# Openflight-sim/OPEN_Ludwig

Measured on AMD Instinct MI355X. Metric: MLUPS (million lattice updates/s) at 256^3 D3Q27; % of HBM roofline, higher is better.
Workload: dtype f32

## Files before the change

open_ludwig_amd/build.py:

```python
from __future__ import annotations

import os
import shutil
import subprocess

_HERE = os.path.dirname(os.path.abspath(__file__))
CSRC = os.path.join(_HERE, "csrc")
SOURCES = ["ludwig_hip.hip"]
DEPENDS = ["ludwig_hip.hip", "kernels.hpp", "all_or_nothing.hpp", "lattice.hpp", "jl_math.h", os.path.join("..", "..", "include", "ludwig_hip.h")]
OUT = os.path.join(CSRC, "libludwig_hip.so")

HIPCC_FLAGS = ["--offload-arch=gfx950", "-O3", "-std=c++17", "-fPIC", "-shared", "-ffp-contract=off",
               "-fno-fast-math", "-Wall", "-Wno-unused-function", "-DLW_NT_STORES"]


def source_digest() -> str:
    import hashlib
    h = hashlib.sha1(" ".join(HIPCC_FLAGS).encode())
    for d in sorted(DEPENDS):
        with open(os.path.join(CSRC, d), "rb") as fh:
            h.update(fh.read())
    return h.hexdigest()[:16]


def hipcc_path() -> str:
    for cand in (shutil.which("hipcc"), "/opt/rocm/bin/hipcc"):
        if cand and os.path.exists(cand):
            return cand
    raise FileNotFoundError("hipcc not found")


def needs_build() -> bool:
    if not os.path.exists(OUT):
        return True
    t = os.path.getmtime(OUT)
    return any(os.path.getmtime(os.path.join(CSRC, d)) > t for d in DEPENDS)


def build_library(force: bool = False, verbose: bool = False, extra_flags=()) -> str:
    if not force and not needs_build():
        return OUT
    cmd = [hipcc_path(), *HIPCC_FLAGS, *extra_flags, *SOURCES, "-o", OUT]
    res = subprocess.run(cmd, cwd=CSRC, capture_output=True, text=True)
    if verbose or res.returncode != 0:
        print(" ".join(cmd))
        print(res.stdout)
        print(res.stderr)
    if res.returncode != 0:
        raise RuntimeError("hipcc failed building libludwig_hip.so")
    return OUT
```

open_ludwig_amd/csrc/kernels.hpp:

```cpp
#pragma once

#include <hip/hip_runtime.h>
#include <stdint.h>
#include <type_traits>

#include "lattice.hpp"
#include "jl_math.h"

namespace lw {

struct SCParams {
    const float *f_in;
    float *f_out;
    float *f_post;
    const uint32_t *post_rows;
    const float *vel_in;
    float *vel_out;
    float *rho;
    const uint8_t *obstacle;
    const float *sponge;
    const float *wall_dist;
    const int32_t *meta;
    const int32_t *items;
    const float *pf_new, *pf_old, *prho_new, *prho_old, *pvel_new, *pvel_old;
// ... 142 lines not shown
    int zs[3];
};

__device__ __forceinline__ NeighbourIds load_neighbour_ids(const int32_t *__restrict__ meta, int z)
{
    int nb[27];
#pragma unroll
    for (int d = 0; d < 27; ++d) nb[d] = meta[d];
    NeighbourIds n;
    const bool z_lo = z == 0, z_hi = z == 7;
#pragma unroll
    for (int j = 0; j < 9; ++j) {
        const int lo = nb[j], mid = nb[9 + j], hi = nb[18 + j];
        n.id[0][j] = z_lo ? lo : mid;
        n.id[1][j] = mid;
        n.id[2][j] = z_hi ? hi : mid;
    }
    n.zs[0] = (z - 1) & 7; n.zs[1] = z; n.zs[2] = (z + 1) & 7;
    return n;
}

struct LanePos {
    int x, y;
    bool x0, x7, y0, y7;
};

template <int K>
__device__ __forceinline__ int source_block(const NeighbourIds &n, const LanePos &l)
{
    constexpr int cx = CX(K), cy = CY(K), g = 1 - CZ(K);
    const bool xo = cx == 1 ? l.x0 : (cx == -1 ? l.x7 : false);
    const bool yo = cy == 1 ? l.y0 : (cy == -1 ? l.y7 : false);
    const int c00 = n.id[g][4], cX = n.id[g][4 - cx], cY = n.id[g][4 - 3 * cy], cXY = n.id[g][4 - cx - 3 * cy];
    int sel = c00;
    if constexpr (cx != 0 && cy != 0) sel = xo ? (yo ? cXY : cX) : (yo ? cY : c00);
    else if constexpr (cx != 0) sel = xo ? cX : c00;
    else if constexpr (cy != 0) sel = yo ? cY : c00;
    return sel;
}
constexpr int SUBGRID_NO_OP1 = 0, SUBGRID_NO_DENOM = 1, SUBGRID_FLOOR = 2, SUBGRID_MODEL = 3;
struct WaleState {
    float nu_eddy, s2;
    int code;
};
__device__ __forceinline__ WaleState wale_state(float g11, float g12, float g13, float g21, float g22, float g23, float g31, float g32,
                                                float g33, float c_wale, float nu_bg)
{
    const float gsq11 = g11 * g11 + g12 * g21 + g13 * g31;
    const float gsq12 = g11 * g12 + g12 * g22 + g13 * g32;
    const float gsq13 = g11 * g13 + g12 * g23 + g13 * g33;
    const float gsq21 = g21 * g11 + g22 * g21 + g23 * g31;
    const float gsq22 = g21 * g12 + g22 * g22 + g23 * g32;
    const float gsq23 = g21 * g13 + g22 * g23 + g23 * g33;
    const float gsq31 = g31 * g11 + g32 * g21 + g33 * g31;
    const float gsq32 = g31 * g12 + g32 * g22 + g33 * g32;
    const float gsq33 = g31 * g13 + g32 * g23 + g33 * g33;

    const float tr_gsq = gsq11 + gsq22 + gsq33;
    const float tr_term = tr_gsq / 3.0f;
    const float Sd11 = gsq11 - tr_term, Sd22 = gsq22 - tr_term, Sd33 = gsq33 - tr_term;
    const float Sd12 = 0.5f * (gsq12 + gsq21), Sd13 = 0.5f * (gsq13 + gsq31), Sd23 = 0.5f * (gsq23 + gsq32);
    const float S12 = 0.5f * (g12 + g21), S13 = 0.5f * (g13 + g31), S23 = 0.5f * (g23 + g32);
    const float OP1 = Sd11 * Sd11 + Sd22 * Sd22 + Sd33 * Sd33 + 2.0f * (Sd12 * Sd12 + Sd13 * Sd13 + Sd23 * Sd23);
    const float OP2 = g11 * g11 + g22 * g22 + g33 * g33 + 2.0f * (S12 * S12 + S13 * S13 + S23 * S23);

    WaleState w;
    w.code = SUBGRID_NO_OP1;
    float nu_eddy = 0.0f;
    if (OP1 > 1.0e-12f) {
        const float OP1_32 = OP1 * sqrtf(OP1);
        const float OP2_52 = OP2 * OP2 * sqrtf(jl_max(OP2, 1.0e-12f));
        const float denom = OP2_52 + OP1 * sqrtf(sqrtf(jl_max(OP1, 1.0e-12f)));
        w.code = SUBGRID_NO_DENOM;
        if (denom > 1.0e-12f) {
            nu_eddy = (c_wale * c_wale) * OP1_32 / denom;
            w.code = nu_eddy > nu_bg ? SUBGRID_MODEL : SUBGRID_FLOOR;
        }
    }
    w.nu_eddy = jl_max(nu_eddy, nu_bg);
    w.s2 = 2.0f * OP2;
    return w;
}

template <int K>
__device__ __forceinline__ float collide_value(float rho, float ux_eq, float uy_eq, float uz_eq, float Pi_xx, float Pi_yy, float Pi_zz,
                                               float Pi_xy, float Pi_yz, float Pi_zx, float one_m_omega)
{
    constexpr int cx = CX(K), cy = CY(K), cz = CZ(K);
    constexpr float w_k = WEIGHT(K);
    constexpr float cx_f = (float)cx, cy_f = (float)cy, cz_f = (float)cz;
    const float usq_eq = ux_eq * ux_eq + uy_eq * uy_eq + uz_eq * uz_eq;
    const float cu = cdot<K>(ux_eq, uy_eq, uz_eq);
    const float feq = rho * w_k * (1.0f + 3.0f * cu + 4.5f * cu * cu - 1.5f * usq_eq);
    constexpr float Q_xx = cx_f * cx_f - CS2_PHYSICS, Q_yy = cy_f * cy_f - CS2_PHYSICS, Q_zz = cz_f * cz_f - CS2_PHYSICS;
    float od = 0.0f;
    bool od_empty = true;
    acc_signed<cx * cy>(od, od_empty, Pi_xy);
    acc_signed<cy * cz>(od, od_empty, Pi_yz);
    acc_signed<cz * cx>(od, od_empty, Pi_zx);
    float inner = Pi_xx * Q_xx + Pi_yy * Q_yy + Pi_zz * Q_zz;
    if constexpr (cx * cy != 0 || cy * cz != 0 || cz * cx != 0) inner = inner + 2.0f * od;
    const float f_neq_reg = (w_k * 4.5f) * inner;
    return feq + one_m_omega * f_neq_reg;
}

constexpr int R_COMP = 11;
constexpr uint32_t R_PLANE_BYTES = R_COMP * 64 * 4, R_BLOCK_BYTES = 8 * R_PLANE_BYTES;
enum { R_RHO, R_UX, R_UY, R_UZ, R_PXX, R_PYY, R_PZZ, R_PXY, R_PYZ, R_PZX, R_OMO };

__device__ __forceinline__ const char *record_plane(const float *base, int blk, int z)
{
    return reinterpret_cast<const char *>(base) + (uint64_t)(uint32_t)blk * R_BLOCK_BYTES + (uint32_t)z * R_PLANE_BYTES;
}
__device__ __forceinline__ void load_record(float (&r)[R_COMP], const char *plane, uint32_t lane4)
{
    const float *q = reinterpret_cast<const float *>(plane + lane4);
#pragma unroll
    for (int c = 0; c < R_COMP; ++c) r[c] = q[c * 64];
}
template <bool WIDE>
using record_off_t = std::conditional_t<WIDE, uint64_t, uint32_t>;
template <bool WIDE>
__device__ __forceinline__ record_off_t<WIDE> record_offset(int blk, int z)
{
    return (record_off_t<WIDE>)(uint32_t)blk * R_BLOCK_BYTES + (uint32_t)z * R_PLANE_BYTES;
}
template <class OFF>
__device__ __forceinline__ void load_record_at(float (&r)[R_COMP], const float *base, OFF off)
{
    const float *q = reinterpret_cast<const float *>(reinterpret_cast<const char *>(base) + off);
#pragma unroll
    for (int c = 0; c < R_COMP; ++c) r[c] = q[c * 64];
}
__device__ __forceinline__ void store_record(float *base, const Own own, float rho, float ux, float uy, float uz, float Pi_xx, float Pi_yy,
                                             float Pi_zz, float Pi_xy, float Pi_yz, float Pi_zx, float one_m_omega)
{
    char *plane = const_cast<char *>(record_plane(base, own.b, __builtin_amdgcn_readfirstlane((int)(own.cell4 >> 8))));
    float *q = reinterpret_cast<float *>(plane + (own.cell4 & 255u));
    const float v[R_COMP] = {rho, ux, uy, uz, Pi_xx, Pi_yy, Pi_zz, Pi_xy, Pi_yz, Pi_zx, one_m_omega};
#pragma unroll
    for (int c = 0; c < R_COMP; ++c) {
#ifdef LW_NT_STORES
        __builtin_nontemporal_store(v[c], q + c * 64);
#else
        q[c * 64] = v[c];
#endif
    }
}
template <int CY_, int CZ_>
__device__ __forceinline__ void record_row(float (&fs)[Q], const float (&r)[R_COMP])
{
    static_for<0, 3>([&](auto ic) {
        constexpr int k = decltype(ic)::value + 3 * (CY_ + 1) + 9 * (CZ_ + 1);
        fs[k] = collide_value<k>(r[R_RHO], r[R_UX], r[R_UY], r[R_UZ], r[R_PXX], r[R_PYY], r[R_PZZ], r[R_PXY], r[R_PYZ], r[R_PZX], r[R_OMO]);
    });
}
template <int CY_, int CZ_>
__device__ __forceinline__ float record_face(const float (&r)[R_COMP], bool plus)
{
    constexpr int k = 2 + 3 * (CY_ + 1) + 9 * (CZ_ + 1);
    return collide_value<k>(r[R_RHO], plus ? r[R_UX] : -r[R_UX], r[R_UY], r[R_UZ], r[R_PXX], r[R_PYY], r[R_PZZ],
                            plus ? r[R_PXY] : -r[R_PXY], r[R_PYZ], plus ? r[R_PZX] : -r[R_PZX], r[R_OMO]);
}

template <bool POST, bool WALL, bool REC_OUT = false>
__device__ __forceinline__ void finish_cell(const SCParams &p, const int flags, const Own own, float (&fs)[Q],
                                            const float ux_E, const float uy_E, const float uz_E, const float ux_W, const float uy_W, const float uz_W,
                                            const float ux_N, const float uy_N, const float uz_N, const float ux_S, const float uy_S, const float uz_S,
                                            const float ux_T, const float uy_T, const float uz_T, const float ux_B, const float uy_B, const float uz_B)
{
    float rho = 0.0f, jx = 0.0f, jy = 0.0f, jz = 0.0f;
    static_for<0, Q>([&](auto kc) {
        constexpr int k = decltype(kc)::value;
        constexpr int cx = CX(k), cy = CY(k), cz = CZ(k);
        const float val = fs[k];
        rho += val;
        if constexpr (cx == 1) jx += val; else if constexpr (cx == -1) jx -= val;
        if constexpr (cy == 1) jy += val; else if constexpr (cy == -1) jy -= val;
        if constexpr (cz == 1) jz += val; else if constexpr (cz == -1) jz -= val;
    });

    bool store_post = false;
    if constexpr (POST) {
        if (flags & FLAG_STORE_POST) {
            store_post = true;
            if (p.post_rows) {
                const int zu = __builtin_amdgcn_readfirstlane((int)(own.cell4 >> 8));
                const uint32_t w = p.post_rows[(size_t)own.b * 2 + (zu >> 2)];
                store_post = ((w >> ((zu & 3) * 8 + ((own.cell4 >> 5) & 7))) & 1u) != 0;
            }
        }
    }
    bool is_obs = false;
    if (flags & FLAG_HAS_OBSTACLE) is_obs = p.obstacle[(size_t)own.b * CELLS + (own.cell4 >> 2)] != 0;
    if (is_obs) {
        st_f32(p.vel_out, own.b, V_BLOCK_BYTES, own.cell4, 0.0f);
        st_f32(p.vel_out, own.b, V_BLOCK_BYTES, COMP_BYTES + own.cell4, 0.0f);
        st_f32(p.vel_out, own.b, V_BLOCK_BYTES, 2 * COMP_BYTES + own.cell4, 0.0f);
        if (p.rho_old_save) st_f32(p.rho_old_save, own.b, S_BLOCK_BYTES, own.cell4, ld_own(p.rho, own.b, S_BLOCK_BYTES, own.cell4));
        if (p.store_rho) st_f32(p.rho, own.b, S_BLOCK_BYTES, own.cell4, 1.0f);
        static_for<0, Q>([&](auto kc) {
            constexpr int k = decltype(kc)::value;
            const float f_coll = fs[OPP(k)];
            st_f32(p.f_out, own.b, F_BLOCK_BYTES, k * COMP_BYTES + own.cell4, f_coll);
            if constexpr (POST) { if (store_post) st_f32(p.f_post, own.b, F_BLOCK_BYTES, k * COMP_BYTES + own.cell4, f_coll); }
        });
        return;
    }

    rho = jl_max(rho, 0.01f);
    const float inv_rho = 1.0f / rho;
    float ux = jx * inv_rho, uy = jy * inv_rho, uz = jz * inv_rho;

    if (flags & FLAG_HAS_SPONGE) {
        const float sp = ld_own(p.sponge, own.b, S_BLOCK_BYTES, own.cell4);
        if (sp > 0.0f) {
            const float rho_target = 1.0f, ux_target = p.u_inlet;
            rho = rho * (1.0f - sp) + rho_target * sp;
            ux = ux * (1.0f - sp) + ux_target * sp;
            uy = uy * (1.0f - sp);
            uz = uz * (1.0f - sp);
            if (p.sponge_blend == 1) {
                static_for<0, Q>([&](auto kc) {
                    constexpr int k = decltype(kc)::value;
                    const float feq_target = calculate_equilibrium(rho_target, ux_target, 0.0f, 0.0f, WEIGHT(k),
                                                                   (float)CX(k), (float)CY(k), (float)CZ(k));
                    fs[k] = fs[k] * (1.0f - sp) + feq_target * sp;
                });
            }
        }
    }

    float Fx = 0.0f, Fy = 0.0f, Fz = 0.0f;
    float ux_eq = ux, uy_eq = uy, uz_eq = uz;
    if constexpr (WALL) {
        if (flags & FLAG_HAS_NEAR_WALL) {
            const float u_mag = sqrtf(ux * ux + uy * uy + uz * uz);
            const float force_mag = wall_model_force_mag(ld_own(p.wall_dist, own.b, S_BLOCK_BYTES, own.cell4), p.tau, rho, u_mag);
            if (force_mag >= 0.0f) {
                Fx = -force_mag * ux / u_mag;
                Fy = -force_mag * uy / u_mag;
                Fz = -force_mag * uz / u_mag;
            }
        }
        ux_eq = ux + 0.5f * Fx * inv_rho;
        uy_eq = uy + 0.5f * Fy * inv_rho;
        uz_eq = uz + 0.5f * Fz * inv_rho;
    }
    const float usq_eq = ux_eq * ux_eq + uy_eq * uy_eq + uz_eq * uz_eq;

    if constexpr (!REC_OUT) {
        st_f32(p.vel_out, own.b, V_BLOCK_BYTES, own.cell4, ux);
        st_f32(p.vel_out, own.b, V_BLOCK_BYTES, COMP_BYTES + own.cell4, uy);
        st_f32(p.vel_out, own.b, V_BLOCK_BYTES, 2 * COMP_BYTES + own.cell4, uz);
        if (p.rho_old_save) st_f32(p.rho_old_save, own.b, S_BLOCK_BYTES, own.cell4, ld_own(p.rho, own.b, S_BLOCK_BYTES, own.cell4));
        if (p.store_rho) st_f32(p.rho, own.b, S_BLOCK_BYTES, own.cell4, rho);
    }

    const float g11 = 0.5f * (ux_E - ux_W), g12 = 0.5f * (ux_N - ux_S), g13 = 0.5f * (ux_T - ux_B);
    const float g21 = 0.5f * (uy_E - uy_W), g22 = 0.5f * (uy_N - uy_S), g23 = 0.5f * (uy_T - uy_B);
    const float g31 = 0.5f * (uz_E - uz_W), g32 = 0.5f * (uz_N - uz_S), g33 = 0.5f * (uz_T - uz_B);

    const float gsq11 = g11 * g11 + g12 * g21 + g13 * g31;
    const float gsq12 = g11 * g12 + g12 * g22 + g13 * g32;
    const float gsq13 = g11 * g13 + g12 * g23 + g13 * g33;
    const float gsq21 = g21 * g11 + g22 * g21 + g23 * g31;
    const float gsq22 = g21 * g12 + g22 * g22 + g23 * g32;
    const float gsq23 = g21 * g13 + g22 * g23 + g23 * g33;
    const float gsq31 = g31 * g11 + g32 * g21 + g33 * g31;
    const float gsq32 = g31 * g12 + g32 * g22 + g33 * g32;
    const float gsq33 = g31 * g13 + g32 * g23 + g33 * g33;

    const float tr_gsq = gsq11 + gsq22 + gsq33;
    const float tr_term = tr_gsq / 3.0f;
    const float Sd11 = gsq11 - tr_term, Sd22 = gsq22 - tr_term, Sd33 = gsq33 - tr_term;
    const float Sd12 = 0.5f * (gsq12 + gsq21), Sd13 = 0.5f * (gsq13 + gsq31), Sd23 = 0.5f * (gsq23 + gsq32);
    const float S12 = 0.5f * (g12 + g21), S13 = 0.5f * (g13 + g31), S23 = 0.5f * (g23 + g32);
    const float OP1 = Sd11 * Sd11 + Sd22 * Sd22 + Sd33 * Sd33 + 2.0f * (Sd12 * Sd12 + Sd13 * Sd13 + Sd23 * Sd23);
    const float OP2 = g11 * g11 + g22 * g22 + g33 * g33 + 2.0f * (S12 * S12 + S13 * S13 + S23 * S23);

    float nu_eddy = 0.0f;
    if (OP1 > 1.0e-12f) {
        const float OP1_32 = OP1 * sqrtf(OP1);
        const float OP2_52 = OP2 * OP2 * sqrtf(jl_max(OP2, 1.0e-12f));
        const float denom = OP2_52 + OP1 * sqrtf(sqrtf(jl_max(OP1, 1.0e-12f)));
        if (denom > 1.0e-12f) nu_eddy = (p.c_wale * p.c_wale) * OP1_32 / denom;
    }
    nu_eddy = jl_max(nu_eddy, p.nu_bg);
    const float tau_turb = p.tau + nu_eddy * 3.0f;
    const float omega = 1.0f / jl_max(tau_turb, 0.500001f);

    float Pi_xx = 0.0f, Pi_yy = 0.0f, Pi_zz = 0.0f, Pi_xy = 0.0f, Pi_yz = 0.0f, Pi_zx = 0.0f;
    static_for<0, Q>([&](auto kc) {
        constexpr int k = decltype(kc)::value;
        constexpr int cx = CX(k), cy = CY(k), cz = CZ(k);
        const float cu = cdot<k>(ux_eq, uy_eq, uz_eq);
        const float feq = rho * WEIGHT(k) * (1.0f + 3.0f * cu + 4.5f * cu * cu - 1.5f * usq_eq);
        const float f_neq = fs[k] - feq;
        if constexpr (cx != 0) Pi_xx += f_neq;
        if constexpr (cy != 0) Pi_yy += f_neq;
        if constexpr (cz != 0) Pi_zz += f_neq;
        if constexpr (cx * cy == 1) Pi_xy += f_neq; else if constexpr (cx * cy == -1) Pi_xy -= f_neq;
        if constexpr (cy * cz == 1) Pi_yz += f_neq; else if constexpr (cy * cz == -1) Pi_yz -= f_neq;
        if constexpr (cz * cx == 1) Pi_zx += f_neq; else if constexpr (cz * cx == -1) Pi_zx -= f_neq;
    });

    const float one_m_omega = 1.0f - omega;
    const float one_m_half_omega = 1.0f - 0.5f * omega;
    if constexpr (REC_OUT) {
        store_record(p.rec_out, own, rho, ux_eq, uy_eq, uz_eq, Pi_xx, Pi_yy, Pi_zz, Pi_xy, Pi_yz, Pi_zx, one_m_omega);
        return;
    }
    static_for<0, Q>([&](auto kc) {
        constexpr int k = decltype(kc)::value;
        float f_coll = collide_value<k>(rho, ux_eq, uy_eq, uz_eq, Pi_xx, Pi_yy, Pi_zz, Pi_xy, Pi_yz, Pi_zx, one_m_omega);
        if constexpr (WALL) {
            constexpr float w_k = WEIGHT(k);
            constexpr float cx_f = (float)CX(k), cy_f = (float)CY(k), cz_f = (float)CZ(k);
            const float cu = cdot<k>(ux_eq, uy_eq, uz_eq);
            const float force_term = (w_k * 3.0f) * ((cx_f - ux + 3.0f * cu * cx_f) * Fx + (cy_f - uy + 3.0f * cu * cy_f) * Fy +
                                                     (cz_f - uz + 3.0f * cu * cz_f) * Fz);
            f_coll = f_coll + one_m_half_omega * force_term;
        }
        if constexpr (POST) { if (store_post) st_f32(p.f_post, own.b, F_BLOCK_BYTES, k * COMP_BYTES + own.cell4, f_coll); }
        st_f32(p.f_out, own.b, F_BLOCK_BYTES, k * COMP_BYTES + own.cell4, f_coll);
    });
}

__device__ __forceinline__ void finish_rho_only(const SCParams &p, const int flags, const Own own, const float (&fs)[Q])
{
    float rho = 0.0f;
    static_for<0, Q>([&](auto kc) { rho += fs[decltype(kc)::value]; });
    bool is_obs = false;
    if (flags & FLAG_HAS_OBSTACLE) is_obs = p.obstacle[(size_t)own.b * CELLS + (own.cell4 >> 2)] != 0;
    if (is_obs) { st_f32(p.rho, own.b, S_BLOCK_BYTES, own.cell4, 1.0f); return; }
    rho = jl_max(rho, 0.01f);
    if (flags & FLAG_HAS_SPONGE) {
        const float sp = ld_own(p.sponge, own.b, S_BLOCK_BYTES, own.cell4);
        if (sp > 0.0f) rho = rho * (1.0f - sp) + 1.0f * sp;
    }
    st_f32(p.rho, own.b, S_BLOCK_BYTES, own.cell4, rho);
}

__device__ __forceinline__ void patch_missing_sources(const SCParams &p, const int32_t *__restrict__ meta, const NeighbourIds &nbr,
                                                      const LanePos &l, const int z, const Own own, float (&fs)[Q])
{
    const int gx = (meta[NBR_BX] - 1) * BS + l.x + 1, gy = (meta[NBR_BY] - 1) * BS + l.y + 1, gz = (meta[NBR_BZ] - 1) * BS + z + 1;
    const float *iface_own = p.is_level_1 == 0 ? p.f_iface + (size_t)meta[NBR_GBI] * CELLS + (own.cell4 >> 2) : nullptr;
    static_for<0, Q>([&](auto kc) {
        constexpr int k = decltype(kc)::value;
        constexpr int cx = CX(k), cy = CY(k), cz = CZ(k);
        if constexpr (k != 13) {
            if (source_block<k>(nbr, l) < 0) {
                const int src_gx = gx - cx, src_gy = gy - cy, src_gz = gz - cz;
                const bool is_inlet = src_gx < 1, is_outlet = src_gx > p.nx_g;
                const bool is_y_min = src_gy < 1, is_y_max = src_gy > p.ny_g;
                const bool is_z_min = src_gz < 1, is_z_max = src_gz > p.nz_g;
                float val;
                if (is_inlet) {
                    const float noise = p.inlet_turbulence > 0.0f
                                            ? gradient_noise(gy, gz, p.seed, 1234) * p.inlet_turbulence * p.u_inlet
                                            : 0.0f;
                    const float u_inst = p.u_inlet + noise;
                    const float cu_in = (float)cx * u_inst;
                    val = WEIGHT(k) * (1.0f + 3.0f * cu_in + 4.5f * cu_in * cu_in - 1.5f * u_inst * u_inst);
                } else if (is_outlet) {
                    const float cu_out = (float)cx * p.u_inlet;
                    val = WEIGHT(k) * (1.0f + 3.0f * cu_out + 4.5f * cu_out * cu_out - 1.5f * p.u_inlet * p.u_inlet);
                } else if (is_y_min && p.is_symmetric == 1) {
                    val = ld_own(p.f_in, own.b, F_BLOCK_BYTES, MIRROR_Y(k) * COMP_BYTES + own.cell4);
                } else if (is_y_min || is_y_max) {
                    val = ld_own(p.f_in, own.b, F_BLOCK_BYTES, MIRROR_Y(k) * COMP_BYTES + own.cell4);
                } else if (is_z_min || is_z_max) {
                    val = ld_own(p.f_in, own.b, F_BLOCK_BYTES, MIRROR_Z(k) * COMP_BYTES + own.cell4);
                } else if (p.is_level_1 == 0) {
                    val = iface_own[(size_t)k * p.n_iface_blocks * CELLS];
                } else {
                    val = WEIGHT(k);
                }
                fs[k] = val;
            }
        }
    });
}

__device__ __forceinline__ float dpp_from_lower_lane(float v)
{
    return __int_as_float(__builtin_amdgcn_update_dpp(__float_as_int(v), __float_as_int(v), 0x111, 0xF, 0xF, false));
// ... 95 lines not shown
            if (l.x7) xch[wave][18 + c][l.y] = uc[c];
            if (l.x0) xch[wave][21 + c][l.y] = uc[c];
        }
    }
    }
    __syncthreads();
    if (!active) return;
    const int wlo = first ? 0 : wave - 1, whi = last ? NW - 1 : wave + 1;
    static_for<0, Q>([&](auto kc) {
        constexpr int k = decltype(kc)::value;
        constexpr int cx = CX(k);
        if constexpr (cx == 1) {
            const float inner = dpp_from_lower_lane(fs[k]);
            const float edge = first ? halo[k] : xch[wlo][XSLOT(k)][l.y];
            fs[k] = l.x0 ? edge : inner;
        }
        if constexpr (cx == -1) {
            const float inner = dpp_from_upper_lane(fs[k]);
            const float edge = last ? halo[k] : xch[whi][XSLOT(k)][l.y];
            fs[k] = l.x7 ? edge : inner;
        }
    });
    const bool needs_patch = GENERAL && (flags & FLAG_ALL_NEIGHBOURS) == 0;
    if constexpr (RHO_ONLY) {
        if constexpr (GENERAL) { if (needs_patch) patch_missing_sources(p, meta, nbr, l, z, own, fs); }
        finish_rho_only(p, flags, own, fs);
        return;
    }
    float uE[3], uW[3], uN[3], uS[3];
#pragma unroll
    for (int c = 0; c < 3; ++c) {
        const float e_edge = last ? ux_edge_hi[c] : xch[whi][21 + c][l.y];
        const float w_edge = first ? ux_edge_lo[c] : xch[wlo][18 + c][l.y];
        const float e_in = dpp_from_upper_lane(uc[c]), w_in = dpp_from_lower_lane(uc[c]);
        uE[c] = l.x7 ? e_edge : e_in;
        uW[c] = l.x0 ? w_edge : w_in;
        const float n_in = __shfl_down(uc[c], 8, 64), s_in = __shfl_up(uc[c], 8, 64);
        uN[c] = l.y7 ? uy_edge[c] : n_in;
        uS[c] = l.y0 ? uy_edge[c] : s_in;
    }
    if constexpr (GENERAL) { if (needs_patch) patch_missing_sources(p, meta, nbr, l, z, own, fs); }
    finish_cell<POST, WALL, REC_OUT>(p, flags, own, fs, uE[0], uE[1], uE[2], uW[0], uW[1], uW[2], uN[0], uN[1], uN[2], uS[0], uS[1], uS[2],
                                     uT[0], uT[1], uT[2], uB[0], uB[1], uB[2]);
}
template <int NW, bool GENERAL, bool POST, bool WALL, bool RHO_ONLY = false, bool WIDE = false>
__global__ __launch_bounds__(64 * NW) __attribute__((amdgpu_waves_per_eu((WIDE && GENERAL) ? LW_MIN_WAVES - 1 : LW_MIN_WAVES))) void k_stream_collide_xrun(const SCParams p)
{
    stream_collide_xrun<NW, GENERAL, POST, WALL, RHO_ONLY, WIDE, false>(p);
}
template <int NW, bool WIDE>
__global__ __launch_bounds__(64 * NW) __attribute__((amdgpu_waves_per_eu(LW_MIN_WAVES))) void k_records_from_populations(const SCParams p)
{
    stream_collide_xrun<NW, false, false, false, false, WIDE, true>(p);
}

#ifndef LW_REC_WAVES
#define LW_REC_WAVES 4
#endif
#ifndef LW_REC_AHEAD
#define LW_REC_AHEAD 3
#endif
template <int NW, bool WIDE>
__global__ __launch_bounds__(64 * NW) __attribute__((amdgpu_waves_per_eu(LW_REC_WAVES))) void k_step_records(const SCParams p)
{
    __shared__ float xch[NW][24][8];
    const int wave = __builtin_amdgcn_readfirstlane(threadIdx.x >> 6);
    const int raw = p.items[blockIdx.x * NW + wave];
    const bool active = raw >= 0;
    const int item = active ? (raw & ITEM_ID_MASK) : 0;
    const int b = item >> 3;
    const int z = item & 7;
    const int lane = threadIdx.x & 63;
    LanePos l;
    l.x = lane & 7; l.y = lane >> 3;
    l.x0 = l.x == 0; l.x7 = l.x == 7; l.y0 = l.y == 0; l.y7 = l.y == 7;
    const int32_t *__restrict__ meta = p.meta + (size_t)b * NBR_STRIDE;
    const NeighbourIds nbr = load_neighbour_ids(meta, z);
    const Own own{b, (uint32_t)((l.x + 8 * l.y + 64 * z) * 4)};
    const bool first = !active || (raw & ITEM_LINK_W) == 0, last = !active || (raw & ITEM_LINK_E) == 0;
    __shared__ float xedge[NW][2][12][8];
    float fs[Q];
    float uc[3], uT[3], uB[3], uN[3], uS[3];
    if (active) {
    if ((first && l.x0) || (last && l.x7)) {
        float r[9][R_COMP];
        auto load_face = [&](auto jc) {
            constexpr int j = decltype(jc)::value;
            constexpr int cy = j % 3 - 1, g = 1 - (j / 3 - 1);
            const bool yo = cy == 1 ? l.y0 : (cy == -1 ? l.y7 : false);
            const int wX = nbr.id[g][4 - 1], wXY = nbr.id[g][4 - 1 - 3 * cy], eX = nbr.id[g][4 + 1], eXY = nbr.id[g][4 + 1 - 3 * cy];
            const auto oW = record_offset<WIDE>(wX, nbr.zs[g]), oWY = record_offset<WIDE>(wXY, nbr.zs[g]);
            const auto oE = record_offset<WIDE>(eX, nbr.zs[g]), oEY = record_offset<WIDE>(eXY, nbr.zs[g]);
            const auto off = l.x0 ? (yo ? oWY : oW) : (yo ? oEY : oE);
            load_record_at(r[j], p.rec_in, off + (uint32_t)(((l.x0 ? 7 : 0) + 8 * ((l.y - cy) & 7)) * 4));
        };
        static_for<0, LW_REC_AHEAD>(load_face);
        static_for<0, 9>([&](auto jc) {
            constexpr int j = decltype(jc)::value;
            constexpr int cy = j % 3 - 1, cz = j / 3 - 1;
            if constexpr (j + LW_REC_AHEAD < 9) load_face(std::integral_constant<int, j + LW_REC_AHEAD>{});
            __builtin_amdgcn_sched_barrier(0);
            float(&mine)[12][8] = xedge[wave][l.x0 ? 0 : 1];
            mine[j][l.y] = record_face<cy, cz>(r[j], l.x0);
            if constexpr (cy == 0 && cz == 0) { mine[9][l.y] = r[j][R_UX]; mine[10][l.y] = r[j][R_UY]; mine[11][l.y] = r[j][R_UZ]; }
            __builtin_amdgcn_sched_barrier(0);
        });
    }
    {
        float r[9][R_COMP];
        auto load_pulled = [&](auto jc) {
            constexpr int j = decltype(jc)::value;
            constexpr int cy = j % 3 - 1, g = 1 - (j / 3 - 1);
            const uint32_t lane4 = (uint32_t)((l.x + 8 * ((l.y - cy) & 7)) * 4);
            if constexpr (cy == 0) {
                load_record(r[j], record_plane(p.rec_in, nbr.id[g][4], nbr.zs[g]), lane4);
            } else {
                const bool yo = cy == 1 ? l.y0 : l.y7;
                const auto o0 = record_offset<WIDE>(nbr.id[g][4], nbr.zs[g]), oY = record_offset<WIDE>(nbr.id[g][4 - 3 * cy], nbr.zs[g]);
                load_record_at(r[j], p.rec_in, (yo ? oY : o0) + lane4);
            }
        };
        static_for<0, LW_REC_AHEAD>(load_pulled);
        static_for<0, 9>([&](auto jc) {
            constexpr int j = decltype(jc)::value;
            constexpr int cy = j % 3 - 1, cz = j / 3 - 1;
            if constexpr (j + LW_REC_AHEAD < 9) load_pulled(std::integral_constant<int, j + LW_REC_AHEAD>{});
            __builtin_amdgcn_sched_barrier(0);
            const float(&q)[R_COMP] = r[j];
            record_row<cy, cz>(fs, q);
            if constexpr (cy == 0 && cz == 0) { uc[0] = q[R_UX]; uc[1] = q[R_UY]; uc[2] = q[R_UZ]; }
            if constexpr (cy == 0 && cz == 1) { uB[0] = q[R_UX]; uB[1] = q[R_UY]; uB[2] = q[R_UZ]; }
            if constexpr (cy == 0 && cz == -1) { uT[0] = q[R_UX]; uT[1] = q[R_UY]; uT[2] = q[R_UZ]; }
            if constexpr (cy == 1 && cz == 0) { uS[0] = q[R_UX]; uS[1] = q[R_UY]; uS[2] = q[R_UZ]; }
            if constexpr (cy == -1 && cz == 0) { uN[0] = q[R_UX]; uN[1] = q[R_UY]; uN[2] = q[R_UZ]; }
            __builtin_amdgcn_sched_barrier(0);
        });
    }
    static_for<0, Q>([&](auto kc) {
        constexpr int k = decltype(kc)::value;
        constexpr int cx = CX(k);
        if constexpr (cx == 1) { if (l.x7) xch[wave][XSLOT(k)][l.y] = fs[k]; }
        if constexpr (cx == -1) { if (l.x0) xch[wave][XSLOT(k)][l.y] = fs[k]; }
    });
#pragma unroll
    for (int c = 0; c < 3; ++c) {
        if (l.x7) xch[wave][18 + c][l.y] = uc[c];
        if (l.x0) xch[wave][21 + c][l.y] = uc[c];
    }
    }
    __syncthreads();
    if (!active) return;
    const int wlo = first ? 0 : wave - 1, whi = last ? NW - 1 : wave + 1;
    static_for<0, Q>([&](auto kc) {
        constexpr int k = decltype(kc)::value;
        constexpr int cx = CX(k);
        if constexpr (cx == 1) {
            const float inner = dpp_from_lower_lane(fs[k]);
            const float edge = first ? xedge[wave][0][k / 3][l.y] : xch[wlo][XSLOT(k)][l.y];
            fs[k] = l.x0 ? edge : inner;
        }
        if constexpr (cx == -1) {
            const float inner = dpp_from_upper_lane(fs[k]);
            const float edge = last ? xedge[wave][1][k / 3][l.y] : xch[whi][XSLOT(k)][l.y];
            fs[k] = l.x7 ? edge : inner;
        }
    });
    float uE[3], uW[3];
#pragma unroll
    for (int c = 0; c < 3; ++c) {
        const float e_edge = last ? xedge[wave][1][9 + c][l.y] : xch[whi][21 + c][l.y];
        const float w_edge = first ? xedge[wave][0][9 + c][l.y] : xch[wlo][18 + c][l.y];
        const float e_in = dpp_from_upper_lane(uc[c]), w_in = dpp_from_lower_lane(uc[c]);
        uE[c] = l.x7 ? e_edge : e_in;
        uW[c] = l.x0 ? w_edge : w_in;
    }
    finish_cell<false, false, true>(p, 0, own, fs, uE[0], uE[1], uE[2], uW[0], uW[1], uW[2], uN[0], uN[1], uN[2], uS[0], uS[1], uS[2],
                                    uT[0], uT[1], uT[2], uB[0], uB[1], uB[2]);
}

__global__ __launch_bounds__(256) void k_materialise(const SCParams p, int64_t n_cells)
{
    const int64_t i = (int64_t)blockIdx.x * 256 + threadIdx.x;
    if (i >= n_cells) return;
    const int b = (int)(i >> 9);
    const uint32_t cell = (uint32_t)(i & 511);
    float r[R_COMP];
    load_record(r, record_plane(p.rec_in, b, (int)(cell >> 6)), (cell & 63u) * 4);
    const Own own{b, cell * 4};
    st_f32(p.vel_out, b, V_BLOCK_BYTES, own.cell4, r[R_UX]);
    st_f32(p.vel_out, b, V_BLOCK_BYTES, COMP_BYTES + own.cell4, r[R_UY]);
    st_f32(p.vel_out, b, V_BLOCK_BYTES, 2 * COMP_BYTES + own.cell4, r[R_UZ]);
    if (p.rho) st_f32(p.rho, b, S_BLOCK_BYTES, own.cell4, r[R_RHO]);
    static_for<0, Q>([&](auto kc) {
        constexpr int k = decltype(kc)::value;
        st_f32(p.f_out, b, F_BLOCK_BYTES, k * COMP_BYTES + own.cell4,
               collide_value<k>(r[R_RHO], r[R_UX], r[R_UY], r[R_UZ], r[R_PXX], r[R_PYY], r[R_PZZ], r[R_PXY], r[R_PYZ], r[R_PZX], r[R_OMO]));
    });
}

__device__ __forceinline__ float weight_rt(int k)
{
    const int cx = k % 3 - 1, cy = (k / 3) % 3 - 1, cz = k / 9 - 1;
    const int d2 = cx * cx + cy * cy + cz * cz;
    return d2 == 0 ? WEIGHT(13) : d2 == 1 ? WEIGHT(12) : d2 == 2 ? WEIGHT(9) : WEIGHT(0);
}

struct InterfaceArgs {
    const int4 *corners;
    const float4 *weights;
    float4 *mac, *mac2;
    const int4 *links;
    float *f_iface2;
    float tw2;
    int n_sources, n_links;
};

__device__ __forceinline__ float blend_in_time(bool blend, float v_old, float v_new, float tw)
{
    return blend ? v_old * (1.0f - tw) + v_new * tw : v_new;
}

template <bool TWO>
__global__ __launch_bounds__(256) void k_interface_sources(const SCParams p, const InterfaceArgs a)
{
    const int i = blockIdx.x * 256 + threadIdx.x;
    if (i >= a.n_sources) return;
    const int4 c0 = a.corners[2 * i], c1 = a.corners[2 * i + 1];
    const int cc[8] = {c0.x, c0.y, c0.z, c0.w, c1.x, c1.y, c1.z, c1.w};
    const float4 w = a.weights[i];
    const float tw = p.temporal_weight, tw2 = a.tw2;
    const bool blend = p.use_temporal == 1 && tw < 0.99f, blend2 = TWO && p.use_temporal == 1 && tw2 < 0.99f;
    float v1[4][8], v2[4][8];
#pragma unroll
    for (int n = 0; n < 8; ++n) {
        v1[0][n] = 1.0f; v1[1][n] = 0.0f; v1[2][n] = 0.0f; v1[3][n] = 0.0f;
        v2[0][n] = 1.0f; v2[1][n] = 0.0f; v2[2][n] = 0.0f; v2[3][n] = 0.0f;
        if (cc[n] >= 0) {
            const int c = cc[n];
            const size_t cv = (size_t)(c >> 9) * (3 * CELLS) + (c & 511);
            const float vn[4] = {p.prho_new[c], p.pvel_new[cv], p.pvel_new[cv + CELLS], p.pvel_new[cv + 2 * CELLS]};
            float vo[4] = {0.0f, 0.0f, 0.0f, 0.0f};
            if (blend || blend2) { vo[0] = p.prho_old[c]; vo[1] = p.pvel_old[cv]; vo[2] = p.pvel_old[cv + CELLS]; vo[3] = p.pvel_old[cv + 2 * CELLS]; }
#pragma unroll
            for (int q = 0; q < 4; ++q) {
                v1[q][n] = blend_in_time(blend, vo[q], vn[q], tw);
                if (TWO) v2[q][n] = blend_in_time(blend2, vo[q], vn[q], tw2);
            }
        }
    }
#pragma unroll
    for (int n = 1; n < 8; ++n)
        if (cc[n] < 0) {
#pragma unroll
            for (int q = 0; q < 4; ++q) { v1[q][n] = v1[q][0]; v2[q][n] = v2[q][0]; }
        }
#define LW_TL(v, q) trilin(v[q][0], v[q][1], v[q][2], v[q][3], v[q][4], v[q][5], v[q][6], v[q][7], w.x, w.y, w.z)
    a.mac[i] = make_float4(LW_TL(v1, 0), LW_TL(v1, 1), LW_TL(v1, 2), LW_TL(v1, 3));
    if (TWO) a.mac2[i] = make_float4(LW_TL(v2, 0), LW_TL(v2, 1), LW_TL(v2, 2), LW_TL(v2, 3));
#undef LW_TL
// ... 1553 lines not shown
```

Before: 24490.

## Pack moment sums into f32x2 and spread x-face record loads across lanes

Moment accumulations (rho/j and the Pi tensor) are regrouped into paired f32x2 chains so the compiler can emit packed FMA/add instructions, and opposite-direction equilibria are computed together. The x-face halo reconstruction, previously done serially by the x0/x7 lanes over 9 directions, is now distributed across lanes via a runtime DirLaneFace descriptor, with one leftover direction handled by the edge lanes. SLP vectorization is disabled to keep control over packing. This trades divergent serial edge work for more uniform per-lane work, at the risk of extra runtime selects and higher register pressure.

```diff
diff --git a/open_ludwig_amd/build.py b/open_ludwig_amd/build.py
--- a/open_ludwig_amd/build.py
+++ b/open_ludwig_amd/build.py
@@ -11,7 +11,7 @@
 OUT = os.path.join(CSRC, "libludwig_hip.so")
 
 HIPCC_FLAGS = ["--offload-arch=gfx950", "-O3", "-std=c++17", "-fPIC", "-shared", "-ffp-contract=off",
-               "-fno-fast-math", "-Wall", "-Wno-unused-function", "-DLW_NT_STORES"]
+               "-fno-fast-math", "-fno-slp-vectorize", "-Wall", "-Wno-unused-function", "-DLW_NT_STORES"]
 
 
 def source_digest() -> str:
diff --git a/open_ludwig_amd/csrc/kernels.hpp b/open_ludwig_amd/csrc/kernels.hpp
--- a/open_ludwig_amd/csrc/kernels.hpp
+++ b/open_ludwig_amd/csrc/kernels.hpp
@@ -248,26 +248,106 @@
     return w;
 }
 
+typedef float f32x2 __attribute__((ext_vector_type(2)));
+
+template <class T>
+__device__ __forceinline__ T equilibrium_value(float rho, float w_k, T cu, float usq_eq)
+{
+    return rho * w_k * (1.0f + 3.0f * cu + 4.5f * cu * cu - 1.5f * usq_eq);
+}
+
+template <bool PACKED>
+struct Chain2;
+template <>
+struct Chain2<true> {
+    f32x2 v = {0.0f, 0.0f};
+    __device__ __forceinline__ void add_both(float a, float b) { v += f32x2{a, b}; }
+    __device__ __forceinline__ void add_first(float a) { v.x += a; }
+    __device__ __forceinline__ void add_second(float b) { v.y += b; }
+    __device__ __forceinline__ float first() const { return v.x; }
+    __device__ __forceinline__ float second() const { return v.y; }
+};
+template <>
+struct Chain2<false> {
+    float s0 = 0.0f, s1 = 0.0f;
+    __device__ __forceinline__ void add_both(float a, float b) { s0 += a; s1 += b; }
+    __device__ __forceinline__ void add_first(float a) { s0 += a; }
+    __device__ __forceinline__ void add_second(float b) { s1 += b; }
+    __device__ __forceinline__ float first() const { return s0; }
+    __device__ __forceinline__ float second() const { return s1; }
+};
+
+template <int K>
+struct DirConst {
+    static constexpr int cx = CX(K), cy = CY(K), cz = CZ(K);
+    __device__ __forceinline__ float weight() const { return WEIGHT(K); }
+    __device__ __forceinline__ float q_xx() const { return (float)cx * (float)cx - CS2_PHYSICS; }
+    __device__ __forceinline__ float q_yy() const { return (float)cy * (float)cy - CS2_PHYSICS; }
+    __device__ __forceinline__ float q_zz() const { return (float)cz * (float)cz - CS2_PHYSICS; }
+    __device__ __forceinline__ float dot(float a, float b, float c) const { return cdot<K>(a, b, c); }
+    __device__ __forceinline__ float add_off_diagonal(float inner, float xy, float yz, float zx) const
+    {
+        float od = 0.0f;
+        bool od_empty = true;
+        acc_signed<cx * cy>(od, od_empty, xy);
+        acc_signed<cy * cz>(od, od_empty, yz);
+        acc_signed<cz * cx>(od, od_empty, zx);
+        if constexpr (cx * cy != 0 || cy * cz != 0 || cz * cx != 0) inner = inner + 2.0f * od;
+        return inner;
+    }
+};
+__device__ __forceinline__ void acc_signed_lane(int c, float &sum, bool &empty, float v)
+{
+    const float t = c > 0 ? v : -v;
+    const float next = empty ? t : sum + t;
+    sum = c != 0 ? next : sum;
+    empty = empty && c == 0;
+}
+struct DirLaneFace {
+    int cy, cz;
+    __device__ __forceinline__ float weight() const
+    {
+        const int n = (cy != 0 ? 1 : 0) + (cz != 0 ? 1 : 0);
+        return n == 0 ? WEIGHT(DIR(1, 0, 0)) : (n == 1 ? WEIGHT(DIR(1, 1, 0)) : WEIGHT(DIR(1, 1, 1)));
+    }
+    __device__ __forceinline__ float q_xx() const { return 1.0f * 1.0f - CS2_PHYSICS; }
+    __device__ __forceinline__ float q_yy() const { return cy != 0 ? 1.0f * 1.0f - CS2_PHYSICS : 0.0f * 0.0f - CS2_PHYSICS; }
+    __device__ __forceinline__ float q_zz() const { return cz != 0 ? 1.0f * 1.0f - CS2_PHYSICS : 0.0f * 0.0f - CS2_PHYSICS; }
+    __device__ __forceinline__ float dot(float a, float b, float c) const
+    {
+        float s = a;
+        bool empty = false;
+        acc_signed_lane(cy, s, empty, b);
+        acc_signed_lane(cz, s, empty, c);
+        return s;
+    }
+    __device__ __forceinline__ float add_off_diagonal(float inner, float xy, float yz, float zx) const
+    {
+        float od = 0.0f;
+        bool od_empty = true;
+        acc_signed_lane(cy, od, od_empty, xy);
+        acc_signed_lane(cy * cz, od, od_empty, yz);
+        acc_signed_lane(cz, od, od_empty, zx);
+        return od_empty ? inner : inner + 2.0f * od;
+    }
+};
+template <class DIRECTION>
+__device__ __forceinline__ float collide_value(const DIRECTION d, float rho, float ux_eq, float uy_eq, float uz_eq, float Pi_xx, float Pi_yy,
+                                               float Pi_zz, float Pi_xy, float Pi_yz, float Pi_zx, float one_m_omega)
+{
+    const float w_k = d.weight();
+    const float usq_eq = ux_eq * ux_eq + uy_eq * uy_eq + uz_eq * uz_eq;
+    const float cu = d.dot(ux_eq, uy_eq, uz_eq);
+    const float feq = equilibrium_value<float>(rho, w_k, cu, usq_eq);
+    const float inner = d.add_off_diagonal(Pi_xx * d.q_xx() + Pi_yy * d.q_yy() + Pi_zz * d.q_zz(), Pi_xy, Pi_yz, Pi_zx);
+    const float f_neq_reg = (w_k * 4.5f) * inner;
+    return feq + one_m_omega * f_neq_reg;
+}
 template <int K>
 __device__ __forceinline__ float collide_value(float rho, float ux_eq, float uy_eq, float uz_eq, float Pi_xx, float Pi_yy, float Pi_zz,
                                                float Pi_xy, float Pi_yz, float Pi_zx, float one_m_omega)
 {
-    constexpr int cx = CX(K), cy = CY(K), cz = CZ(K);
-    constexpr float w_k = WEIGHT(K);
-    constexpr float cx_f = (float)cx, cy_f = (float)cy, cz_f = (float)cz;
-    const float usq_eq = ux_eq * ux_eq + uy_eq * uy_eq + uz_eq * uz_eq;
-    const float cu = cdot<K>(ux_eq, uy_eq, uz_eq);
-    const float feq = rho * w_k * (1.0f + 3.0f * cu + 4.5f * cu * cu - 1.5f * usq_eq);
-    constexpr float Q_xx = cx_f * cx_f - CS2_PHYSICS, Q_yy = cy_f * cy_f - CS2_PHYSICS, Q_zz = cz_f * cz_f - CS2_PHYSICS;
-    float od = 0.0f;
-    bool od_empty = true;
-    acc_signed<cx * cy>(od, od_empty, Pi_xy);
-    acc_signed<cy * cz>(od, od_empty, Pi_yz);
-    acc_signed<cz * cx>(od, od_empty, Pi_zx);
-    float inner = Pi_xx * Q_xx + Pi_yy * Q_yy + Pi_zz * Q_zz;
-    if constexpr (cx * cy != 0 || cy * cz != 0 || cz * cx != 0) inner = inner + 2.0f * od;
-    const float f_neq_reg = (w_k * 4.5f) * inner;
-    return feq + one_m_omega * f_neq_reg;
+    return collide_value(DirConst<K>{}, rho, ux_eq, uy_eq, uz_eq, Pi_xx, Pi_yy, Pi_zz, Pi_xy, Pi_yz, Pi_zx, one_m_omega);
 }
 
 constexpr int R_COMP = 11;
@@ -321,30 +401,32 @@
         fs[k] = collide_value<k>(r[R_RHO], r[R_UX], r[R_UY], r[R_UZ], r[R_PXX], r[R_PYY], r[R_PZZ], r[R_PXY], r[R_PYZ], r[R_PZX], r[R_OMO]);
     });
 }
-template <int CY_, int CZ_>
-__device__ __forceinline__ float record_face(const float (&r)[R_COMP], bool plus)
-{
-    constexpr int k = 2 + 3 * (CY_ + 1) + 9 * (CZ_ + 1);
-    return collide_value<k>(r[R_RHO], plus ? r[R_UX] : -r[R_UX], r[R_UY], r[R_UZ], r[R_PXX], r[R_PYY], r[R_PZZ],
-                            plus ? r[R_PXY] : -r[R_PXY], r[R_PYZ], plus ? r[R_PZX] : -r[R_PZX], r[R_OMO]);
-}
-
-template <bool POST, bool WALL, bool REC_OUT = false>
+template <class DIRECTION>
+__device__ __forceinline__ float record_face(const DIRECTION d, const float (&r)[R_COMP], bool plus)
+{
+    return collide_value(d, r[R_RHO], plus ? r[R_UX] : -r[R_UX], r[R_UY], r[R_UZ], r[R_PXX], r[R_PYY], r[R_PZZ],
+                         plus ? r[R_PXY] : -r[R_PXY], r[R_PYZ], plus ? r[R_PZX] : -r[R_PZX], r[R_OMO]);
+}
+
+template <bool POST, bool WALL, bool REC_OUT = false, bool PACKED = false>
 __device__ __forceinline__ void finish_cell(const SCParams &p, const int flags, const Own own, float (&fs)[Q],
                                             const float ux_E, const float uy_E, const float uz_E, const float ux_W, const float uy_W, const float uz_W,
                                             const float ux_N, const float uy_N, const float uz_N, const float ux_S, const float uy_S, const float uz_S,
                                             const float ux_T, const float uy_T, const float uz_T, const float ux_B, const float uy_B, const float uz_B)
 {
-    float rho = 0.0f, jx = 0.0f, jy = 0.0f, jz = 0.0f;
+    Chain2<PACKED> m_rx, m_yz;
     static_for<0, Q>([&](auto kc) {
         constexpr int k = decltype(kc)::value;
         constexpr int cx = CX(k), cy = CY(k), cz = CZ(k);
         const float val = fs[k];
-        rho += val;
-        if constexpr (cx == 1) jx += val; else if constexpr (cx == -1) jx -= val;
-        if constexpr (cy == 1) jy += val; else if constexpr (cy == -1) jy -= val;
-        if constexpr (cz == 1) jz += val; else if constexpr (cz == -1) jz -= val;
+        if constexpr (cx != 0) m_rx.add_both(val, cx > 0 ? val : -val);
+        else m_rx.add_first(val);
+        if constexpr (cy != 0 && cz != 0) m_yz.add_both(cy > 0 ? val : -val, cz > 0 ? val : -val);
+        else if constexpr (cy != 0) m_yz.add_first(cy > 0 ? val : -val);
+        else if constexpr (cz != 0) m_yz.add_second(cz > 0 ? val : -val);
     });
+    float rho = m_rx.first();
+    const float jx = m_rx.second(), jy = m_yz.first(), jz = m_yz.second();
 
     bool store_post = false;
     if constexpr (POST) {
@@ -456,20 +538,29 @@
     const float tau_turb = p.tau + nu_eddy * 3.0f;
     const float omega = 1.0f / jl_max(tau_turb, 0.500001f);
 
-    float Pi_xx = 0.0f, Pi_yy = 0.0f, Pi_zz = 0.0f, Pi_xy = 0.0f, Pi_yz = 0.0f, Pi_zx = 0.0f;
+    Chain2<PACKED> P_x, P_y, P_z;
     static_for<0, Q>([&](auto kc) {
-        constexpr int k = decltype(kc)::value;
+        constexpr int k = decltype(kc)::value, ko = OPP(k);
         constexpr int cx = CX(k), cy = CY(k), cz = CZ(k);
-        const float cu = cdot<k>(ux_eq, uy_eq, uz_eq);
-        const float feq = rho * WEIGHT(k) * (1.0f + 3.0f * cu + 4.5f * cu * cu - 1.5f * usq_eq);
-        const float f_neq = fs[k] - feq;
-        if constexpr (cx != 0) Pi_xx += f_neq;
-        if constexpr (cy != 0) Pi_yy += f_neq;
-        if constexpr (cz != 0) Pi_zz += f_neq;
-        if constexpr (cx * cy == 1) Pi_xy += f_neq; else if constexpr (cx * cy == -1) Pi_xy -= f_neq;
-        if constexpr (cy * cz == 1) Pi_yz += f_neq; else if constexpr (cy * cz == -1) Pi_yz -= f_neq;
-        if constexpr (cz * cx == 1) Pi_zx += f_neq; else if constexpr (cz * cx == -1) Pi_zx -= f_neq;
+        float f_neq;
+        if constexpr (PACKED && k < ko) {
+            const float cu = cdot<k>(ux_eq, uy_eq, uz_eq);
+            const f32x2 both = f32x2{fs[k], fs[ko]} - equilibrium_value<f32x2>(rho, WEIGHT(k), f32x2{cu, -cu}, usq_eq);
+            f_neq = both.x;
+            fs[ko] = both.y;
+        } else if constexpr (PACKED && k > ko) {
+            f_neq = fs[k];
+        } else {
+            f_neq = fs[k] - equilibrium_value<float>(rho, WEIGHT(k), cdot<k>(ux_eq, uy_eq, uz_eq), usq_eq);
+        }
+        if constexpr (cx * cy != 0) P_x.add_both(f_neq, cx * cy > 0 ? f_neq : -f_neq);
+        else if constexpr (cx != 0) P_x.add_first(f_neq);
+        if constexpr (cy * cz != 0) P_y.add_both(f_neq, cy * cz > 0 ? f_neq : -f_neq);
+        else if constexpr (cy != 0) P_y.add_first(f_neq);
+        if constexpr (cz * cx != 0) P_z.add_both(f_neq, cz * cx > 0 ? f_neq : -f_neq);
+        else if constexpr (cz != 0) P_z.add_first(f_neq);
     });
+    const float Pi_xx = P_x.first(), Pi_xy = P_x.second(), Pi_yy = P_y.first(), Pi_yz = P_y.second(), Pi_zz = P_z.first(), Pi_zx = P_z.second();
 
     const float one_m_omega = 1.0f - omega;
     const float one_m_half_omega = 1.0f - 0.5f * omega;
@@ -731,30 +822,37 @@
     float fs[Q];
     float uc[3], uT[3], uB[3], uN[3], uS[3];
     if (active) {
+    auto face_rows = [&](auto sc) {
+        constexpr int side = decltype(sc)::value;
+        constexpr int jx = side == 0 ? 4 - 1 : 4 + 1;
+        const int j = l.x;
+        const int jz = (j >= 3 ? 1 : 0) + (j >= 6 ? 1 : 0);
+        const int cy = j - 3 * jz - 1, cz = jz - 1, g = 2 - jz;
+        auto by_g = [&](int v0, int v1, int v2) { return g == 0 ? v0 : (g == 1 ? v1 : v2); };
+        const int bX = by_g(nbr.id[0][jx], nbr.id[1][jx], nbr.id[2][jx]);
+        const int bXlo = by_g(nbr.id[0][jx - 3], nbr.id[1][jx - 3], nbr.id[2][jx - 3]);
+        const int bXhi = by_g(nbr.id[0][jx + 3], nbr.id[1][jx + 3], nbr.id[2][jx + 3]);
+        const int blk = (cy == 1 && l.y0) ? bXlo : ((cy == -1 && l.y7) ? bXhi : bX);
+        const int zsrc = by_g(nbr.zs[0], nbr.zs[1], nbr.zs[2]);
+        float r[R_COMP];
+        load_record_at(r, p.rec_in, record_offset<WIDE>(blk, zsrc) + (uint32_t)(((side == 0 ? 7 : 0) + 8 * ((l.y - cy) & 7)) * 4));
+        float(&mine)[12][8] = xedge[wave][side];
+        mine[j][l.y] = record_face(DirLaneFace{cy, cz}, r, side == 0);
+        if (j == 4) { mine[9][l.y] = r[R_UX]; mine[10][l.y] = r[R_UY]; mine[11][l.y] = r[R_UZ]; }
+    };
+    if (first) face_rows(std::integral_constant<int, 0>{});
+    if (last) face_rows(std::integral_constant<int, 1>{});
     if ((first && l.x0) || (last && l.x7)) {
-        float r[9][R_COMP];
-        auto load_face = [&](auto jc) {
-            constexpr int j = decltype(jc)::value;
-            constexpr int cy = j % 3 - 1, g = 1 - (j / 3 - 1);
-            const bool yo = cy == 1 ? l.y0 : (cy == -1 ? l.y7 : false);
-            const int wX = nbr.id[g][4 - 1], wXY = nbr.id[g][4 - 1 - 3 * cy], eX = nbr.id[g][4 + 1], eXY = nbr.id[g][4 + 1 - 3 * cy];
-            const auto oW = record_offset<WIDE>(wX, nbr.zs[g]), oWY = record_offset<WIDE>(wXY, nbr.zs[g]);
-            const auto oE = record_offset<WIDE>(eX, nbr.zs[g]), oEY = record_offset<WIDE>(eXY, nbr.zs[g]);
-            const auto off = l.x0 ? (yo ? oWY : oW) : (yo ? oEY : oE);
-            load_record_at(r[j], p.rec_in, off + (uint32_t)(((l.x0 ? 7 : 0) + 8 * ((l.y - cy) & 7)) * 4));
-        };
-        static_for<0, LW_REC_AHEAD>(load_face);
-        static_for<0, 9>([&](auto jc) {
-            constexpr int j = decltype(jc)::value;
-            constexpr int cy = j % 3 - 1, cz = j / 3 - 1;
-            if constexpr (j + LW_REC_AHEAD < 9) load_face(std::integral_constant<int, j + LW_REC_AHEAD>{});
-            __builtin_amdgcn_sched_barrier(0);
-            float(&mine)[12][8] = xedge[wave][l.x0 ? 0 : 1];
-            mine[j][l.y] = record_face<cy, cz>(r[j], l.x0);
-            if constexpr (cy == 0 && cz == 0) { mine[9][l.y] = r[j][R_UX]; mine[10][l.y] = r[j][R_UY]; mine[11][l.y] = r[j][R_UZ]; }
-            __builtin_amdgcn_sched_barrier(0);
-        });
-    }
+        constexpr int j = 8, cy = 1, g = 0;
+        const int wX = nbr.id[g][4 - 1], wXY = nbr.id[g][4 - 1 - 3 * cy], eX = nbr.id[g][4 + 1], eXY = nbr.id[g][4 + 1 - 3 * cy];
+        const auto oW = record_offset<WIDE>(wX, nbr.zs[g]), oWY = record_offset<WIDE>(wXY, nbr.zs[g]);
+        const auto oE = record_offset<WIDE>(eX, nbr.zs[g]), oEY = record_offset<WIDE>(eXY, nbr.zs[g]);
+        const auto off = l.x0 ? (l.y0 ? oWY : oW) : (l.y0 ? oEY : oE);
+        float r[R_COMP];
+        load_record_at(r, p.rec_in, off + (uint32_t)(((l.x0 ? 7 : 0) + 8 * ((l.y - cy) & 7)) * 4));
+        xedge[wave][l.x0 ? 0 : 1][j][l.y] = record_face(DirConst<DIR(1, 1, 1)>{}, r, l.x0);
+    }
+    __builtin_amdgcn_sched_barrier(0);
     {
         float r[9][R_COMP];
         auto load_pulled = [&](auto jc) {
@@ -823,7 +921,7 @@
         uE[c] = l.x7 ? e_edge : e_in;
         uW[c] = l.x0 ? w_edge : w_in;
     }
-    finish_cell<false, false, true>(p, 0, own, fs, uE[0], uE[1], uE[2], uW[0], uW[1], uW[2], uN[0], uN[1], uN[2], uS[0], uS[1], uS[2],
+    finish_cell<false, false, true, true>(p, 0, own, fs, uE[0], uE[1], uE[2], uW[0], uW[1], uW[2], uN[0], uN[1], uN[2], uS[0], uS[1], uS[2],
                                     uT[0], uT[1], uT[2], uB[0], uB[1], uB[2]);
 }
 
```

Result: faster. 25930 (median of 6 runs) (+5.9%).
